# Picsart-AI-Research/StreamingT2V

Measured on NVIDIA H100. Metric: denoise_steps_per_sec, higher is better.
Workload: dtype bf16

## Files before the change

### streamingt2v_b200/csrc/flash_attn.cu

```cuda
#include <cuda.h>
#include <cuda_bf16.h>
#include <math.h>

#include "../../include/b200svd.h"
#include "common.h"
#include "ptx.cuh"
#include "wgmma.cuh"

namespace b200 {

constexpr int FA_BQ = 128;
constexpr int FA_BK = 128;
constexpr int FA_KV_STAGES = 4;
constexpr int FA_THREADS = 3 * 128;
constexpr int FA_WIDE_BYTES = 128 * 64 * 2;

constexpr int fa_tile_bytes(int D) { return 128 * D * 2; }
constexpr int fa_smem_bytes(int D) { return fa_tile_bytes(D) + FA_KV_STAGES * 2 * fa_tile_bytes(D) + 256; }

struct FaParams {
  __nv_bfloat16* out;
  int64_t ldo;
  int S, C;
  float scale_log2;
};

template <int D>
__device__ __forceinline__ void flash_attn_body(const CUtensorMap& tmW, const CUtensorMap& tmT, const FaParams& p) {
  static_assert(D == 64 || D == 80, "head dim 64, or 64 + one 16-column tail");
  constexpr int TAIL = D - 64;
  constexpr int TAIL_BYTES = 128 * TAIL * 2;
  constexpr int TILE_BYTES = fa_tile_bytes(D);

  extern __shared__ __align__(1024) uint8_t smem[];
  if ((smem_u32(smem) & 1023u) != 0) __trap();
  uint8_t* sQ = smem;
  uint8_t* sKV = sQ + TILE_BYTES;
  uint64_t* bars = reinterpret_cast<uint64_t*>(sKV + FA_KV_STAGES * 2 * TILE_BYTES);
  uint64_t* q_full = bars;
  uint64_t* kv_full = bars + 1;
  uint64_t* kv_empty = kv_full + FA_KV_STAGES;

  const int warp = threadIdx.x >> 5, lane = threadIdx.x & 31;
  const int wg = warp >> 2;
  const int head = blockIdx.y, n = blockIdx.z;
  const int q0 = blockIdx.x * FA_BQ;
  const int nkb = (p.S + FA_BK - 1) / FA_BK;

  if (threadIdx.x == 0) {
    prefetch_tmap(&tmW);
    if constexpr (TAIL > 0) prefetch_tmap(&tmT);
    mbar_init(q_full, 1);
    for (int s = 0; s < FA_KV_STAGES; ++s) {
      mbar_init(&kv_full[s], 1);
      mbar_init(&kv_empty[s], 2);
    }
    fence_barrier_init();
  }
  __syncthreads();

  if (wg == 0) {
    asm volatile("setmaxnreg.dec.sync.aligned.u32 40;");
    if (threadIdx.x == 0) {
      const int col = head * D;
      mbar_expect_tx(q_full, TILE_BYTES);
      tma_load_3d(sQ, &tmW, q_full, col, q0, n);
      if constexpr (TAIL > 0) tma_load_3d(sQ + FA_WIDE_BYTES, &tmT, q_full, col + 64, q0, n);
      for (int j = 0; j < nkb; ++j) {
        const int s = j % FA_KV_STAGES;
        mbar_wait_parked(&kv_empty[s], ((j / FA_KV_STAGES) & 1) ^ 1);
        uint8_t* sk = sKV + s * 2 * TILE_BYTES;
        uint8_t* sv = sk + TILE_BYTES;
        mbar_expect_tx(&kv_full[s], 2 * TILE_BYTES);
        tma_load_3d(sk, &tmW, &kv_full[s], p.C + col, j * FA_BK, n);
        if constexpr (TAIL > 0) tma_load_3d(sk + FA_WIDE_BYTES, &tmT, &kv_full[s], p.C + col + 64, j * FA_BK, n);
        tma_load_3d(sv, &tmW, &kv_full[s], 2 * p.C + col, j * FA_BK, n);
        if constexpr (TAIL > 0) tma_load_3d(sv + FA_WIDE_BYTES, &tmT, &kv_full[s], 2 * p.C + col + 64, j * FA_BK, n);
      }
    }
    return;
  }
  asm volatile("setmaxnreg.inc.sync.aligned.u32 232;");

  const int cw = wg - 1, wl = warp & 3;
  const int rq = lane >> 2, cq = lane & 3;
  const float c = p.scale_log2;
  const uint64_t qdesc = smem_desc_k_sw128(smem_u32(sQ + cw * (FA_WIDE_BYTES / 2)));
  const uint64_t qdesc_t = smem_desc_k_sw32(smem_u32(sQ + FA_WIDE_BYTES + cw * (TAIL_BYTES / 2)));
  float o[32];
  float ot[TAIL > 0 ? TAIL / 2 : 1];
#pragma unroll
  for (int i = 0; i < 32; ++i) o[i] = 0.f;
#pragma unroll
  for (int i = 0; i < TAIL / 2; ++i) ot[i] = 0.f;
  float m_run[2] = {-INFINITY, -INFINITY};
  float l_run[2] = {0.f, 0.f};
  mbar_wait(q_full, 0);

  for (int j = 0; j < nkb; ++j) {
    const int st = j % FA_KV_STAGES;
    mbar_wait(&kv_full[st], (j / FA_KV_STAGES) & 1);
    const uint32_t sk = smem_u32(sKV + st * 2 * TILE_BYTES);
    const uint32_t sv = sk + TILE_BYTES;
    float sacc[64];
#pragma unroll
    for (int i = 0; i < 64; ++i) sacc[i] = 0.f;
    wgmma_fence_regs(sacc);
    wgmma_fence();
    const uint64_t kdesc = smem_desc_k_sw128(sk);
#pragma unroll
    for (int kk = 0; kk < 4; ++kk) Wgmma<128>::ss(sacc, qdesc + (uint64_t)(kk * 2), kdesc + (uint64_t)(kk * 2), 1u);
    if constexpr (TAIL > 0) Wgmma<128>::ss(sacc, qdesc_t, smem_desc_k_sw32(sk + FA_WIDE_BYTES), 1u);
    wgmma_commit();
    wgmma_wait<0>();
    wgmma_fence_regs(sacc);

    const int kbase = j * FA_BK;
    if (kbase + FA_BK > p.S) {
#pragma unroll
      for (int jj = 0; jj < 16; ++jj)
#pragma unroll
        for (int e = 0; e < 2; ++e)
          if (kbase + 8 * jj + 2 * cq + e >= p.S) {
            sacc[4 * jj + e] = -INFINITY;
            sacc[4 * jj + 2 + e] = -INFINITY;
          }
    }
    float alpha[2];
#pragma unroll
    for (int h = 0; h < 2; ++h) {
      float mx = -INFINITY;
#pragma unroll
      for (int jj = 0; jj < 16; ++jj) mx = fmaxf(mx, fmaxf(sacc[4 * jj + 2 * h], sacc[4 * jj + 2 * h + 1]));
      mx = fmaxf(mx, __shfl_xor_sync(0xffffffffu, mx, 1));
      mx = fmaxf(mx, __shfl_xor_sync(0xffffffffu, mx, 2));
      const float m_new = fmaxf(m_run[h], mx * c);
      alpha[h] = ex2_approx(m_run[h] - m_new);
      m_run[h] = m_new;
      float l = 0.f;
#pragma unroll
      for (int jj = 0; jj < 16; ++jj) {
#pragma unroll
        for (int e = 0; e < 2; ++e) {
          const float pr = ex2_approx(fmaf(sacc[4 * jj + 2 * h + e], c, -m_new));
          sacc[4 * jj + 2 * h + e] = pr;
          l += pr;
        }
      }
      l_run[h] = l_run[h] * alpha[h] + l;
    }
#pragma unroll
    for (int jj = 0; jj < 8; ++jj) {
      o[4 * jj] *= alpha[0];
      o[4 * jj + 1] *= alpha[0];
      o[4 * jj + 2] *= alpha[1];
      o[4 * jj + 3] *= alpha[1];
    }
#pragma unroll
    for (int jj = 0; jj < TAIL / 8; ++jj) {
      ot[4 * jj] *= alpha[0];
      ot[4 * jj + 1] *= alpha[0];
      ot[4 * jj + 2] *= alpha[1];
      ot[4 * jj + 3] *= alpha[1];
    }
    uint32_t pa[8][4];
#pragma unroll
    for (int kk = 0; kk < 8; ++kk) {
      pa[kk][0] = pack_bf16x2(sacc[8 * kk + 0], sacc[8 * kk + 1]);
      pa[kk][1] = pack_bf16x2(sacc[8 * kk + 2], sacc[8 * kk + 3]);
      pa[kk][2] = pack_bf16x2(sacc[8 * kk + 4], sacc[8 * kk + 5]);
      pa[kk][3] = pack_bf16x2(sacc[8 * kk + 6], sacc[8 * kk + 7]);
    }
    const uint64_t vdesc = smem_desc_mn_sw128(sv);
    const uint64_t vdesc_t = smem_desc_mn_sw32(sv + FA_WIDE_BYTES);
    wgmma_fence_regs(o);
    if constexpr (TAIL > 0) wgmma_fence_regs(ot);
    wgmma_fence();
#pragma unroll
    for (int kk = 0; kk < 8; ++kk) {
      Wgmma<64>::rs_tb(o, pa[kk], vdesc + (uint64_t)(kk * 128), 1u);
      if constexpr (TAIL > 0) Wgmma<TAIL>::rs_tb(ot, pa[kk], vdesc_t + (uint64_t)(kk * 32), 1u);
    }
    wgmma_commit();
    wgmma_wait<0>();
    wgmma_fence_regs(o);
    if constexpr (TAIL > 0) wgmma_fence_regs(ot);
    if ((threadIdx.x & 127) == 0) mbar_arrive(&kv_empty[st]);
  }

#pragma unroll
  for (int h = 0; h < 2; ++h) {
    float l = l_run[h];
    l += __shfl_xor_sync(0xffffffffu, l, 1);
    l += __shfl_xor_sync(0xffffffffu, l, 2);
    const float inv = 1.0f / l;
    const int qrow = q0 + 64 * cw + 16 * wl + rq + 8 * h;
    if (qrow < p.S) {
      __nv_bfloat16* dst = p.out + ((int64_t)n * p.S + qrow) * p.ldo + head * D + 2 * cq;
#pragma unroll
      for (int jj = 0; jj < 8; ++jj)
        *reinterpret_cast<uint32_t*>(dst + 8 * jj) = pack_bf16x2(o[4 * jj + 2 * h] * inv, o[4 * jj + 2 * h + 1] * inv);
#pragma unroll
      for (int jj = 0; jj < TAIL / 8; ++jj)
        *reinterpret_cast<uint32_t*>(dst + 64 + 8 * jj) =
            pack_bf16x2(ot[4 * jj + 2 * h] * inv, ot[4 * jj + 2 * h + 1] * inv);
    }
  }
}

__global__ void __launch_bounds__(FA_THREADS, 1)
flash_attn_kernel(const __grid_constant__ CUtensorMap tmW, const __grid_constant__ CUtensorMap tmT, const FaParams p) {
  flash_attn_body<64>(tmW, tmT, p);
}

__global__ void __launch_bounds__(FA_THREADS, 1)
flash_attn_d80_kernel(const __grid_constant__ CUtensorMap tmW, const __grid_constant__ CUtensorMap tmT,
                      const FaParams p) {
  flash_attn_body<80>(tmW, tmT, p);
}

template <int D>
static int flash_attn_launch(const char* name, const void* qkv, int64_t ldqkv, void* out, int64_t ldo, int n, int s,
                             int heads, float scale, void* stream) {
  if (n <= 0 || s <= 0 || heads <= 0 || n > 65535 || heads > 65535) {
    set_error("%s: need n, s, heads >= 1 (n, heads <= 65535), got n=%d s=%d heads=%d", name, n, s, heads);
    return 1;
  }
  if (ldqkv % 8 || ldo % 8) {
    set_error("%s: leading dims must be multiples of 8", name);
    return 1;
  }
  const int C = heads * D;
  if (ldqkv < 3 * (int64_t)C || ldo < (int64_t)C) {
    set_error("%s: ldqkv (%lld) must be >= 3*heads*%d and ldo (%lld) >= heads*%d (%d)", name, (long long)ldqkv, D,
              (long long)ldo, D, C);
    return 1;
  }
  if ((reinterpret_cast<uintptr_t>(qkv) & 15) != 0 || (reinterpret_cast<uintptr_t>(out) & 15) != 0) {
    set_error("%s: qkv and out must be 16-byte aligned", name);
    return 1;
  }
  CUtensorMap tmW, tmT = {};
  uint64_t dims[3] = {(uint64_t)3 * C, (uint64_t)s, (uint64_t)n};
  uint64_t strides[2] = {(uint64_t)ldqkv * 2, (uint64_t)ldqkv * 2 * (uint64_t)s};
  uint32_t box_w[3] = {64, 128, 1};
  if (encode_tmap_bf16(&tmW, qkv, 3, dims, strides, box_w)) return 1;
  if constexpr (D > 64) {
    uint32_t box_t[3] = {D - 64, 128, 1};
    if (encode_tmap_bf16_sw32(&tmT, qkv, 3, dims, strides, box_t)) return 1;
  }
  auto* kernel = D == 64 ? flash_attn_kernel : flash_attn_d80_kernel;
  static bool attr_set[B200_MAX_DEVICES] = {};
  const int slot = dev_slot();
  if (!attr_set[slot]) {
    cudaError_t e = cudaFuncSetAttribute(kernel, cudaFuncAttributeMaxDynamicSharedMemorySize, fa_smem_bytes(D));
    if (e != cudaSuccess) return cuda_fail(e, name);
    attr_set[slot] = true;
  }
  FaParams p;
  p.out = reinterpret_cast<__nv_bfloat16*>(out);
  p.ldo = ldo;
  p.S = s;
  p.C = C;
  p.scale_log2 = scale * 1.4426950408889634f;
  dim3 grid((s + FA_BQ - 1) / FA_BQ, heads, n);
  kernel<<<grid, FA_THREADS, fa_smem_bytes(D), reinterpret_cast<cudaStream_t>(stream)>>>(tmW, tmT, p);
  B200_CHECK_LAUNCH(name);
  return 0;
}

static int g_fa_variant = 4;

}

extern "C" int b200svd_flash_attn_variant(int v) {
  const int prev = b200::g_fa_variant;
  if (v >= 3 && v <= 5) b200::g_fa_variant = v;
  return prev;
}

extern "C" int b200svd_flash_attn(const void* qkv, int64_t ldqkv, void* out, int64_t ldo, int n, int s, int heads,
                                  float scale, void* stream) {
  return b200::flash_attn_launch<64>("flash_attn", qkv, ldqkv, out, ldo, n, s, heads, scale, stream);
}

extern "C" int b200svd_flash_attn_d80(const void* qkv, int64_t ldqkv, void* out, int64_t ldo, int n, int s, int heads,
                                      float scale, void* stream) {
  return b200::flash_attn_launch<80>("flash_attn_d80", qkv, ldqkv, out, ldo, n, s, heads, scale, stream);
}
```

Measured before the change: 2.542.

## Pipeline QK and PV wgmmas with ping-pong warpgroup scheduling in flash attention

Restructures the consumer loop of the flash attention kernel so the S=QK^T wgmma for the next KV block is issued together with the PV wgmma of the current block, letting softmax overlap with tensor-core work. It adds named-barrier ping-pong between the two consumer warpgroups so they take turns issuing MMAs, and it delays the release of each KV stage by one iteration. The row-max reduction is also rewritten as a tree. The cost is extra live registers and more complex synchronisation, which risks spills or deadlock at the loop edges.

```diff
diff --git a/streamingt2v_b200/csrc/flash_attn.cu b/streamingt2v_b200/csrc/flash_attn.cu
--- a/streamingt2v_b200/csrc/flash_attn.cu
+++ b/streamingt2v_b200/csrc/flash_attn.cu
@@ -13,6 +13,7 @@
 constexpr int FA_BK = 128;
 constexpr int FA_KV_STAGES = 4;
 constexpr int FA_THREADS = 3 * 128;
+constexpr int FA_PINGPONG_THREADS = 2 * 128;
 constexpr int FA_WIDE_BYTES = 128 * 64 * 2;
 
 constexpr int fa_tile_bytes(int D) { return 128 * D * 2; }
@@ -95,16 +96,27 @@
   for (int i = 0; i < TAIL / 2; ++i) ot[i] = 0.f;
   float m_run[2] = {-INFINITY, -INFINITY};
   float l_run[2] = {0.f, 0.f};
+  float sacc[64];
+  uint32_t pa[8][4];
+  float alpha[2];
   mbar_wait(q_full, 0);
 
-  for (int j = 0; j < nkb; ++j) {
-    const int st = j % FA_KV_STAGES;
-    mbar_wait(&kv_full[st], (j / FA_KV_STAGES) & 1);
-    const uint32_t sk = smem_u32(sKV + st * 2 * TILE_BYTES);
-    const uint32_t sv = sk + TILE_BYTES;
-    float sacc[64];
+  const int n_issues = nkb + 1;
+  int issue_no = 0;
+  auto take_turn = [&]() { named_bar_sync(1 + cw, FA_PINGPONG_THREADS); };
+  auto pass_turn = [&]() {
+    if (cw == 0 || ++issue_no < n_issues) named_bar_arrive(2 - cw, FA_PINGPONG_THREADS);
+  };
+  if (cw == 1) named_bar_arrive(1, FA_PINGPONG_THREADS);
+
+  auto wait_kv = [&](int j) {
+    mbar_wait(&kv_full[j % FA_KV_STAGES], (j / FA_KV_STAGES) & 1);
 #pragma unroll
     for (int i = 0; i < 64; ++i) sacc[i] = 0.f;
+  };
+
+  auto issue_s = [&](int j) {
+    const uint32_t sk = smem_u32(sKV + (j % FA_KV_STAGES) * 2 * TILE_BYTES);
     wgmma_fence_regs(sacc);
     wgmma_fence();
     const uint64_t kdesc = smem_desc_k_sw128(sk);
@@ -112,9 +124,30 @@
     for (int kk = 0; kk < 4; ++kk) Wgmma<128>::ss(sacc, qdesc + (uint64_t)(kk * 2), kdesc + (uint64_t)(kk * 2), 1u);
     if constexpr (TAIL > 0) Wgmma<128>::ss(sacc, qdesc_t, smem_desc_k_sw32(sk + FA_WIDE_BYTES), 1u);
     wgmma_commit();
+  };
+
+  auto issue_pv = [&](int j) {
+    const uint32_t sv = smem_u32(sKV + (j % FA_KV_STAGES) * 2 * TILE_BYTES) + TILE_BYTES;
+    const uint64_t vdesc = smem_desc_mn_sw128(sv);
+    const uint64_t vdesc_t = smem_desc_mn_sw32(sv + FA_WIDE_BYTES);
+    wgmma_fence_regs(o);
+    if constexpr (TAIL > 0) wgmma_fence_regs(ot);
+    wgmma_fence();
+#pragma unroll
+    for (int kk = 0; kk < 8; ++kk) {
+      Wgmma<64>::rs_tb(o, pa[kk], vdesc + (uint64_t)(kk * 128), 1u);
+      if constexpr (TAIL > 0) Wgmma<TAIL>::rs_tb(ot, pa[kk], vdesc_t + (uint64_t)(kk * 32), 1u);
+    }
+    wgmma_commit();
+  };
+
+  auto wait_pv = [&]() {
     wgmma_wait<0>();
-    wgmma_fence_regs(sacc);
-
+    wgmma_fence_regs(o);
+    if constexpr (TAIL > 0) wgmma_fence_regs(ot);
+  };
+
+  auto softmax = [&](int j) {
     const int kbase = j * FA_BK;
     if (kbase + FA_BK > p.S) {
 #pragma unroll
@@ -126,15 +159,25 @@
             sacc[4 * jj + 2 + e] = -INFINITY;
           }
     }
-    float alpha[2];
+    float mx[2];
 #pragma unroll
     for (int h = 0; h < 2; ++h) {
-      float mx = -INFINITY;
-#pragma unroll
-      for (int jj = 0; jj < 16; ++jj) mx = fmaxf(mx, fmaxf(sacc[4 * jj + 2 * h], sacc[4 * jj + 2 * h + 1]));
-      mx = fmaxf(mx, __shfl_xor_sync(0xffffffffu, mx, 1));
-      mx = fmaxf(mx, __shfl_xor_sync(0xffffffffu, mx, 2));
-      const float m_new = fmaxf(m_run[h], mx * c);
+      float t[16];
+#pragma unroll
+      for (int jj = 0; jj < 16; ++jj) t[jj] = fmaxf(sacc[4 * jj + 2 * h], sacc[4 * jj + 2 * h + 1]);
+#pragma unroll
+      for (int i = 0; i < 8; ++i) t[i] = fmaxf(t[i], t[i + 8]);
+#pragma unroll
+      for (int i = 0; i < 4; ++i) t[i] = fmaxf(t[i], t[i + 4]);
+      mx[h] = fmaxf(fmaxf(t[0], t[2]), fmaxf(t[1], t[3]));
+    }
+#pragma unroll
+    for (int h = 0; h < 2; ++h) mx[h] = fmaxf(mx[h], __shfl_xor_sync(0xffffffffu, mx[h], 1));
+#pragma unroll
+    for (int h = 0; h < 2; ++h) mx[h] = fmaxf(mx[h], __shfl_xor_sync(0xffffffffu, mx[h], 2));
+#pragma unroll
+    for (int h = 0; h < 2; ++h) {
+      const float m_new = fmaxf(m_run[h], mx[h] * c);
       alpha[h] = ex2_approx(m_run[h] - m_new);
       m_run[h] = m_new;
       float l = 0.f;
@@ -149,6 +192,9 @@
       }
       l_run[h] = l_run[h] * alpha[h] + l;
     }
+  };
+
+  auto rescale_pack = [&]() {
 #pragma unroll
     for (int jj = 0; jj < 8; ++jj) {
       o[4 * jj] *= alpha[0];
@@ -163,7 +209,6 @@
       ot[4 * jj + 2] *= alpha[1];
       ot[4 * jj + 3] *= alpha[1];
     }
-    uint32_t pa[8][4];
 #pragma unroll
     for (int kk = 0; kk < 8; ++kk) {
       pa[kk][0] = pack_bf16x2(sacc[8 * kk + 0], sacc[8 * kk + 1]);
@@ -171,22 +216,36 @@
       pa[kk][2] = pack_bf16x2(sacc[8 * kk + 4], sacc[8 * kk + 5]);
       pa[kk][3] = pack_bf16x2(sacc[8 * kk + 6], sacc[8 * kk + 7]);
     }
-    const uint64_t vdesc = smem_desc_mn_sw128(sv);
-    const uint64_t vdesc_t = smem_desc_mn_sw32(sv + FA_WIDE_BYTES);
-    wgmma_fence_regs(o);
-    if constexpr (TAIL > 0) wgmma_fence_regs(ot);
-    wgmma_fence();
-#pragma unroll
-    for (int kk = 0; kk < 8; ++kk) {
-      Wgmma<64>::rs_tb(o, pa[kk], vdesc + (uint64_t)(kk * 128), 1u);
-      if constexpr (TAIL > 0) Wgmma<TAIL>::rs_tb(ot, pa[kk], vdesc_t + (uint64_t)(kk * 32), 1u);
-    }
-    wgmma_commit();
-    wgmma_wait<0>();
-    wgmma_fence_regs(o);
-    if constexpr (TAIL > 0) wgmma_fence_regs(ot);
-    if ((threadIdx.x & 127) == 0) mbar_arrive(&kv_empty[st]);
-  }
+  };
+
+  wait_kv(0);
+  take_turn();
+  issue_s(0);
+  pass_turn();
+  wgmma_wait<0>();
+  wgmma_fence_regs(sacc);
+  softmax(0);
+  for (int j = 0; j + 1 < nkb; ++j) {
+    wait_pv();
+    if (j > 0 && (threadIdx.x & 127) == 0) mbar_arrive(&kv_empty[(j - 1) % FA_KV_STAGES]);
+    rescale_pack();
+    wait_kv(j + 1);
+    take_turn();
+    issue_s(j + 1);
+    issue_pv(j);
+    pass_turn();
+    wgmma_wait<1>();
+    wgmma_fence_regs(sacc);
+    softmax(j + 1);
+  }
+  wait_pv();
+  if (nkb > 1 && (threadIdx.x & 127) == 0) mbar_arrive(&kv_empty[(nkb - 2) % FA_KV_STAGES]);
+  rescale_pack();
+  take_turn();
+  issue_pv(nkb - 1);
+  pass_turn();
+  wait_pv();
+  if ((threadIdx.x & 127) == 0) mbar_arrive(&kv_empty[(nkb - 1) % FA_KV_STAGES]);
 
 #pragma unroll
   for (int h = 0; h < 2; ++h) {
```

New measurement: 2.587, median of 6. 1.8% higher.

## Overlap QK and PV wgmma across iterations with warpgroup ping-pong scheduling

Applied to the files above, without the earlier changes.

Restructures the flash-attention consumer loop so the QK^T wgmma for block j is issued together with the PV wgmma for block j-1. The softmax of block j then runs while the PV GEMM is still in flight. Named barriers alternate the two consumer warpgroups so their tensor-core issue phases interleave (FA3-style ping-pong), meant to hide softmax latency behind MMA. It also adds an optional polynomial FMA-based exp2 for a configurable fraction of elements to offload the MUFU unit, disabled by default. The cost is more live registers and extra barrier synchronisation.

```diff
diff --git a/streamingt2v_b200/csrc/flash_attn.cu b/streamingt2v_b200/csrc/flash_attn.cu
--- a/streamingt2v_b200/csrc/flash_attn.cu
+++ b/streamingt2v_b200/csrc/flash_attn.cu
@@ -14,6 +14,14 @@
 constexpr int FA_KV_STAGES = 4;
 constexpr int FA_THREADS = 3 * 128;
 constexpr int FA_WIDE_BYTES = 128 * 64 * 2;
+constexpr int FA_BAR_TURN = 1;
+
+#ifndef FA_EXP2_FMA_EIGHTHS_D64
+#define FA_EXP2_FMA_EIGHTHS_D64 0
+#endif
+#ifndef FA_EXP2_FMA_EIGHTHS_D80
+#define FA_EXP2_FMA_EIGHTHS_D80 0
+#endif
 
 constexpr int fa_tile_bytes(int D) { return 128 * D * 2; }
 constexpr int fa_smem_bytes(int D) { return fa_tile_bytes(D) + FA_KV_STAGES * 2 * fa_tile_bytes(D) + 256; }
@@ -25,7 +33,18 @@
   float scale_log2;
 };
 
-template <int D>
+__device__ __forceinline__ float exp2_fma(float x) {
+  constexpr float kRound = 12582912.0f;
+  x = fmaxf(x, -127.0f);
+  const float t = x + kRound;
+  const float f = x - (t - kRound);
+  float p = fmaf(0.05500906f, f, 0.24221097f);
+  p = fmaf(p, f, 0.6932829f);
+  p = fmaf(p, f, 1.0f);
+  return __uint_as_float(__float_as_uint(p) + (__float_as_uint(t) << 23));
+}
+
+template <int D, int FMA_EIGHTHS>
 __device__ __forceinline__ void flash_attn_body(const CUtensorMap& tmW, const CUtensorMap& tmT, const FaParams& p) {
   static_assert(D == 64 || D == 80, "head dim 64, or 64 + one 16-column tail");
   constexpr int TAIL = D - 64;
@@ -95,14 +114,24 @@
   for (int i = 0; i < TAIL / 2; ++i) ot[i] = 0.f;
   float m_run[2] = {-INFINITY, -INFINITY};
   float l_run[2] = {0.f, 0.f};
-  mbar_wait(q_full, 0);
-
-  for (int j = 0; j < nkb; ++j) {
-    const int st = j % FA_KV_STAGES;
-    mbar_wait(&kv_full[st], (j / FA_KV_STAGES) & 1);
-    const uint32_t sk = smem_u32(sKV + st * 2 * TILE_BYTES);
-    const uint32_t sv = sk + TILE_BYTES;
-    float sacc[64];
+  float sacc[64];
+  uint32_t pa[8][4];
+
+  auto issue_pv = [&](int j) {
+    const uint32_t sv = smem_u32(sKV + (j % FA_KV_STAGES) * 2 * TILE_BYTES) + TILE_BYTES;
+    const uint64_t vdesc = smem_desc_mn_sw128(sv);
+    const uint64_t vdesc_t = smem_desc_mn_sw32(sv + FA_WIDE_BYTES);
+    wgmma_fence_regs(o);
+    if constexpr (TAIL > 0) wgmma_fence_regs(ot);
+    wgmma_fence();
+#pragma unroll
+    for (int kk = 0; kk < 8; ++kk) {
+      Wgmma<64>::rs_tb(o, pa[kk], vdesc + (uint64_t)(kk * 128), 1u);
+      if constexpr (TAIL > 0) Wgmma<TAIL>::rs_tb(ot, pa[kk], vdesc_t + (uint64_t)(kk * 32), 1u);
+    }
+  };
+  auto issue_qk = [&](int j) {
+    const uint32_t sk = smem_u32(sKV + (j % FA_KV_STAGES) * 2 * TILE_BYTES);
 #pragma unroll
     for (int i = 0; i < 64; ++i) sacc[i] = 0.f;
     wgmma_fence_regs(sacc);
@@ -111,10 +140,26 @@
 #pragma unroll
     for (int kk = 0; kk < 4; ++kk) Wgmma<128>::ss(sacc, qdesc + (uint64_t)(kk * 2), kdesc + (uint64_t)(kk * 2), 1u);
     if constexpr (TAIL > 0) Wgmma<128>::ss(sacc, qdesc_t, smem_desc_k_sw32(sk + FA_WIDE_BYTES), 1u);
-    wgmma_commit();
+  };
+  auto wait_scores = [&] {
+    wgmma_wait<1>();
+    wgmma_fence_regs(sacc);
+  };
+  auto wait_all = [&] {
     wgmma_wait<0>();
+    wgmma_fence_regs(o);
+    if constexpr (TAIL > 0) wgmma_fence_regs(ot);
     wgmma_fence_regs(sacc);
-
+#pragma unroll
+    for (int kk = 0; kk < 8; ++kk)
+#pragma unroll
+      for (int i = 0; i < 4; ++i) asm volatile("" : "+r"(pa[kk][i])::"memory");
+  };
+  auto release = [&](int j) {
+    if ((threadIdx.x & 127) == 0) mbar_arrive(&kv_empty[j % FA_KV_STAGES]);
+  };
+  auto wait_kv = [&](int j) { mbar_wait(&kv_full[j % FA_KV_STAGES], (j / FA_KV_STAGES) & 1); };
+  auto scores = [&](int j, float (&alpha)[2]) {
     const int kbase = j * FA_BK;
     if (kbase + FA_BK > p.S) {
 #pragma unroll
@@ -126,7 +171,6 @@
             sacc[4 * jj + 2 + e] = -INFINITY;
           }
     }
-    float alpha[2];
 #pragma unroll
     for (int h = 0; h < 2; ++h) {
       float mx = -INFINITY;
@@ -142,13 +186,16 @@
       for (int jj = 0; jj < 16; ++jj) {
 #pragma unroll
         for (int e = 0; e < 2; ++e) {
-          const float pr = ex2_approx(fmaf(sacc[4 * jj + 2 * h + e], c, -m_new));
+          const float x = fmaf(sacc[4 * jj + 2 * h + e], c, -m_new);
+          const float pr = (jj & 7) < FMA_EIGHTHS ? exp2_fma(x) : ex2_approx(x);
           sacc[4 * jj + 2 * h + e] = pr;
           l += pr;
         }
       }
       l_run[h] = l_run[h] * alpha[h] + l;
     }
+  };
+  auto rescale_pack = [&](const float (&alpha)[2]) {
 #pragma unroll
     for (int jj = 0; jj < 8; ++jj) {
       o[4 * jj] *= alpha[0];
@@ -163,7 +210,6 @@
       ot[4 * jj + 2] *= alpha[1];
       ot[4 * jj + 3] *= alpha[1];
     }
-    uint32_t pa[8][4];
 #pragma unroll
     for (int kk = 0; kk < 8; ++kk) {
       pa[kk][0] = pack_bf16x2(sacc[8 * kk + 0], sacc[8 * kk + 1]);
@@ -171,22 +217,40 @@
       pa[kk][2] = pack_bf16x2(sacc[8 * kk + 4], sacc[8 * kk + 5]);
       pa[kk][3] = pack_bf16x2(sacc[8 * kk + 6], sacc[8 * kk + 7]);
     }
-    const uint64_t vdesc = smem_desc_mn_sw128(sv);
-    const uint64_t vdesc_t = smem_desc_mn_sw32(sv + FA_WIDE_BYTES);
-    wgmma_fence_regs(o);
-    if constexpr (TAIL > 0) wgmma_fence_regs(ot);
-    wgmma_fence();
-#pragma unroll
-    for (int kk = 0; kk < 8; ++kk) {
-      Wgmma<64>::rs_tb(o, pa[kk], vdesc + (uint64_t)(kk * 128), 1u);
-      if constexpr (TAIL > 0) Wgmma<TAIL>::rs_tb(ot, pa[kk], vdesc_t + (uint64_t)(kk * 32), 1u);
-    }
+  };
+
+  const int bar_own = FA_BAR_TURN + cw, bar_other = FA_BAR_TURN + (cw ^ 1);
+  float alpha[2];
+  if (cw == 1) named_bar_arrive(bar_other, 256);
+  mbar_wait(q_full, 0);
+  wait_kv(0);
+  named_bar_sync(bar_own, 256);
+  issue_qk(0);
+  wgmma_commit();
+  named_bar_arrive(bar_other, 256);
+  wait_all();
+  scores(0, alpha);
+  rescale_pack(alpha);
+  for (int j = 1; j < nkb; ++j) {
+    wait_kv(j);
+    named_bar_sync(bar_own, 256);
+    issue_qk(j);
     wgmma_commit();
-    wgmma_wait<0>();
-    wgmma_fence_regs(o);
-    if constexpr (TAIL > 0) wgmma_fence_regs(ot);
-    if ((threadIdx.x & 127) == 0) mbar_arrive(&kv_empty[st]);
-  }
+    issue_pv(j - 1);
+    wgmma_commit();
+    named_bar_arrive(bar_other, 256);
+    wait_scores();
+    scores(j, alpha);
+    wait_all();
+    release(j - 1);
+    rescale_pack(alpha);
+  }
+  named_bar_sync(bar_own, 256);
+  issue_pv(nkb - 1);
+  wgmma_commit();
+  if (cw == 0) named_bar_arrive(bar_other, 256);
+  wait_all();
+  release(nkb - 1);
 
 #pragma unroll
   for (int h = 0; h < 2; ++h) {
@@ -210,13 +274,13 @@
 
 __global__ void __launch_bounds__(FA_THREADS, 1)
 flash_attn_kernel(const __grid_constant__ CUtensorMap tmW, const __grid_constant__ CUtensorMap tmT, const FaParams p) {
-  flash_attn_body<64>(tmW, tmT, p);
+  flash_attn_body<64, FA_EXP2_FMA_EIGHTHS_D64>(tmW, tmT, p);
 }
 
 __global__ void __launch_bounds__(FA_THREADS, 1)
 flash_attn_d80_kernel(const __grid_constant__ CUtensorMap tmW, const __grid_constant__ CUtensorMap tmT,
                       const FaParams p) {
-  flash_attn_body<80>(tmW, tmT, p);
+  flash_attn_body<80, FA_EXP2_FMA_EIGHTHS_D80>(tmW, tmT, p);
 }
 
 template <int D>
```

After: 2.558 before, 2.602 after (median of 6 runs). 1.7% higher.
